# westlake-repl/PixelRec

Measured on AMD Instinct MI355X. Metric: user-sequences/sec at emb=512 seq_len=50 (SASRec IDNet training step: fwd+bwd+AdamW), higher is better.
Workload: dtype f32; 1 GPU; BASELINE.json configs[1]: SASRec IDNet emb=512 seq_len=50, 400001 items, 4 heads, inner 2x, 2 layers, BPR loss vs 1 sampled negative, dropout 0.1, AdamW lr 1e-4 wd 0.1; batch_per_gpu=64, global_batch=64, seq_len=50, n_items=400001, embedding_size=512, parallelism=dp1, hip_graph=True

## Files before the change

### pixelrec_amd/csrc/gemm_p3.hip

```cpp
#include "gemm_p4.cuh"

#include <cstdlib>

namespace pxr {

template <int EPI>
__device__ __forceinline__ float p3_epi_elem(float v, float bv, float av, float& aux_out, int act) {
  if constexpr (EPI == EPI_BIAS) {
    v += bv;
  } else if constexpr (EPI == EPI_BIAS_GELU) {
    v += bv;
    aux_out = v;
    v = gelu_erf(v);
  } else if constexpr (EPI == EPI_BIAS_GELU_GRAD) {
    v += bv;
    aux_out = dgelu_erf(v);
    v = gelu_erf(v);
  } else if constexpr (EPI == EPI_MUL) {
    v *= av;
  } else if constexpr (EPI == EPI_MUL_DGELU) {
    v *= dgelu_erf(av);
  } else if constexpr (EPI == EPI_ADD) {
    v += av;
  } else if constexpr (EPI == EPI_BIAS_ADD) {
// ... 105 lines not shown
        apre[it][4] = a1.x; apre[it][5] = a1.y; apre[it][6] = a1.z; apre[it][7] = a1.w;
      }
    }
  }
  float c_scale = 1.0f;
  if constexpr (Cfg::HALF) {
    const int ea = g.a_exp_dev ? *g.a_exp_dev : g.a_exp, eb = g.b_exp_dev ? *g.b_exp_dev : g.b_exp;
    const float sc = ldexpf(1.0f, -(ea + eb));
    if (g.c_exp_dev) c_scale = ldexpf(1.0f, *g.c_exp_dev);
#pragma unroll
    for (int i = 0; i < Cfg::TM; ++i)
#pragma unroll
      for (int j = 0; j < Cfg::TN; ++j)
#pragma unroll
        for (int e = 0; e < 16; ++e) accs.v[i][j][e] *= sc;
  }
  auto chunk = [&](int it, int row, int col, int nv, float (&v)[8]) __attribute__((always_inline)) {
    float bv[8], av[8], ao[8];
    const bool vec = vec_ok && nv == 8;
    if constexpr (EpiTraits<EPI>::HAS_BIAS) {
      if (vec) {
#pragma unroll
        for (int e = 0; e < 8; ++e) bv[e] = bpre[e];
      } else {
#pragma unroll
        for (int e = 0; e < 8; ++e) bv[e] = e < nv ? g.bias[col + e] : 0.f;
      }
    }
    if constexpr (EpiTraits<EPI>::READS_AUX) {
      const float* ap = g.aux + (int64_t)row * g.ldaux + col;
      if (vec) {
        if constexpr (PRE_AUX) {
#pragma unroll
          for (int e = 0; e < 8; ++e) av[e] = apre[it][e];
        } else {
          const float4 a0 = *reinterpret_cast<const float4*>(ap), a1 = *reinterpret_cast<const float4*>(ap + 4);
          av[0] = a0.x; av[1] = a0.y; av[2] = a0.z; av[3] = a0.w; av[4] = a1.x; av[5] = a1.y; av[6] = a1.z; av[7] = a1.w;
        }
      } else {
#pragma unroll
        for (int e = 0; e < 8; ++e) av[e] = e < nv ? ap[e] : 0.f;
      }
    }
#pragma unroll
    for (int e = 0; e < 8; ++e)
      v[e] = p3_epi_elem<EPI>(v[e], EpiTraits<EPI>::HAS_BIAS ? bv[e] : 0.f, EpiTraits<EPI>::READS_AUX ? av[e] : 0.f, ao[e], g.act);
    if (g.dbg & 16) return;
    if constexpr (P3EpiTraits<EPI>::WRITES_AUX) {
      float* ap = g.aux + (int64_t)row * g.ldaux + col;
      if (vec) {
        *reinterpret_cast<float4*>(ap) = make_float4(ao[0], ao[1], ao[2], ao[3]);
        *reinterpret_cast<float4*>(ap + 4) = make_float4(ao[4], ao[5], ao[6], ao[7]);
      } else {
#pragma unroll
        for (int e = 0; e < 8; ++e)
          if (e < nv) ap[e] = ao[e];
      }
    }
    if (g.C != nullptr) {
      float* cp = g.C + (int64_t)row * g.ldc + col;
      if (vec) {
        *reinterpret_cast<float4*>(cp) = make_float4(v[0], v[1], v[2], v[3]);
        *reinterpret_cast<float4*>(cp + 4) = make_float4(v[4], v[5], v[6], v[7]);
      } else {
#pragma unroll
        for (int e = 0; e < 8; ++e)
          if (e < nv) cp[e] = v[e];
      }
    }
    if (g.Cp.p != nullptr) {
      if constexpr (Cfg::HALF) {
#pragma unroll
        for (int e = 0; e < 8; ++e) v[e] *= c_scale;
      }
      px_store8(g.Cp, g.cp_fmt, g.status, row, col, v);
    }
  };
  if constexpr (PP) {
    p4_row_epilogue<Cfg>(accs, smem, g.M, g.N, m0, n0,
                         [&](int it, int row, int col, int nv) {
                           if (!(vec_ok && nv == 8)) return;
                           if constexpr (EpiTraits<EPI>::HAS_BIAS) {
                             if (it == 0) {
                               const float4 b0 = *reinterpret_cast<const float4*>(g.bias + col), b1 = *reinterpret_cast<const float4*>(g.bias + col + 4);
                               bpre[0] = b0.x; bpre[1] = b0.y; bpre[2] = b0.z; bpre[3] = b0.w; bpre[4] = b1.x; bpre[5] = b1.y; bpre[6] = b1.z; bpre[7] = b1.w;
                             }
                           }
                           if constexpr (PRE_AUX) {
                             const float* ap = g.aux + (int64_t)row * g.ldaux + col;
                             const float4 a0 = *reinterpret_cast<const float4*>(ap), a1 = *reinterpret_cast<const float4*>(ap + 4);
                             apre[it][0] = a0.x; apre[it][1] = a0.y; apre[it][2] = a0.z; apre[it][3] = a0.w;
                             apre[it][4] = a1.x; apre[it][5] = a1.y; apre[it][6] = a1.z; apre[it][7] = a1.w;
                           }
                         },
                         chunk);
  } else {
    p3_row_epilogue<Cfg>(accs, smem, g.M, g.N, m0, n0, chunk);
  }
}

__global__ void __launch_bounds__(256) split_planes_kernel(const float* __restrict__ x, int64_t ldx, int64_t rows, int cols8, P3Mat out,
                                                           int xcd) {
  const int64_t i = (int64_t)(xcd ? xcd_remap(blockIdx.x, gridDim.x) : blockIdx.x) * 256 + threadIdx.x;
  if (i >= rows * cols8) return;
  const int64_t row = i / cols8;
  const int c = (int)(i % cols8) * 8;
  const float4 a = *reinterpret_cast<const float4*>(x + row * ldx + c);
  const float4 b = *reinterpret_cast<const float4*>(x + row * ldx + c + 4);
  const float v[8] = {a.x, a.y, a.z, a.w, b.x, b.y, b.z, b.w};
  p3_store8(out, row, c, v);
}

struct P3DwProblem {
  P3Mat dy, x;
  float* dW;
  float* db;
  int T, N, K;
  int tile_begin, tiles_m;
  int dy_exp, x_exp;
  const int* dy_exp_dev;
  const int* x_exp_dev;
};
struct P3DwGroup {
  P3DwProblem p[DW_MAX];
  int n, total_tiles;
  unsigned* flags;
  unsigned* status;
};
int pxr_stream_flags(hipStream_t st, unsigned** flags, int* n_flags);
template <class Cfg, bool EARLY, int KS = 1>
__global__ void __launch_bounds__(Cfg::NT) grouped_dw_p3_kernel(const P3DwGroup g) {
  extern __shared__ __attribute__((aligned(16))) char smem[];
  static_assert(KS == 1 || (KS == 2 && Cfg::PINGPONG), "split-K: the ping-pong tiles");
  const int tl = xcd_remap(blockIdx.x, KS * g.total_tiles);
  const int t = tl / KS, half = tl % KS;
  int pi = 0;
#pragma unroll 1
  for (int i = 1; i < g.n; ++i)
    if (t >= g.p[i].tile_begin) pi = i;
  const P3DwProblem& P = g.p[pi];
  const int local = t - P.tile_begin;
  const int tm = local % P.tiles_m, tn = local / P.tiles_m;
  const int m0 = tm * Cfg::BM, n0 = tn * Cfg::BN;
  const int kpad = (P.T + 31) & ~31;
  typename Cfg::Acc accs;
  f32x16 ones_acc[Cfg::TM];
  const bool do_bias = (P.db != nullptr) && (tn == 0);
  if constexpr (KS == 2) {
    const int k0 = (kpad / 64) * 32;
    const int kb = half ? k0 : 0, kl = half ? kpad - k0 : k0;
    const P3Mat dyh{P.dy.p + (int64_t)kb * 32, P.dy.ps, P.dy.pr}, xh{P.x.p + (int64_t)kb * 32, P.x.ps, P.x.pr};
    if (do_bias) gemm_p4_mainloop<Cfg, false, false, true>(accs, dyh, xh, kl, m0, n0, smem, ones_acc);
    else gemm_p4_mainloop<Cfg, false, false, false>(accs, dyh, xh, kl, m0, n0, smem);
    if (half) {
      if (threadIdx.x == 0) {
        unsigned spins = 0;
        while (__hip_atomic_load(&g.flags[t], __ATOMIC_RELAXED, __HIP_MEMORY_SCOPE_AGENT) == 0u) {
          __builtin_amdgcn_s_sleep(4);
          if (++spins > (1u << 22)) {
            if (g.status) atomicOr(g.status, (unsigned)PXR_STATUS_GEMM_TIMEOUT);
            break;
          }
        }
      }
      __syncthreads();
    }
  } else if constexpr (Cfg::PINGPONG) {
    if (do_bias) gemm_p4_mainloop<Cfg, false, false, true>(accs, P.dy, P.x, kpad, m0, n0, smem, ones_acc);
    else gemm_p4_mainloop<Cfg, false, false, false>(accs, P.dy, P.x, kpad, m0, n0, smem);
  } else {
    if (do_bias) gemm_p3_mainloop<Cfg, false, false, EARLY, true>(accs, P.dy, P.x, kpad, m0, n0, smem, ones_acc);
    else gemm_p3_mainloop<Cfg, false, false, EARLY, false>(accs, P.dy, P.x, kpad, m0, n0, smem);
  }
  if constexpr (Cfg::HALF) {
    const int ey = P.dy_exp_dev ? *P.dy_exp_dev : P.dy_exp, ex = P.x_exp_dev ? *P.x_exp_dev : P.x_exp;
    const float sc = ldexpf(1.0f, -(ey + ex)), sb = ldexpf(1.0f, -ey);
#pragma unroll
    for (int i = 0; i < Cfg::TM; ++i) {
#pragma unroll
      for (int j = 0; j < Cfg::TN; ++j)
#pragma unroll
        for (int e = 0; e < 16; ++e) accs.v[i][j][e] *= sc;
      if (do_bias) {
#pragma unroll
        for (int e = 0; e < 16; ++e) ones_acc[i][e] *= sb;
      }
    }
  }
  float* dW = P.dW;
  const int64_t ldw = P.K;
  const bool vec_ok = (P.K % 8 == 0);
  constexpr int COH = (1 << 4) | 1;
  const bool add = (KS == 2) && half;
  const bool publish = (KS == 2) && !half;
  const bufrsrc rsw = make_rsrc(dW, (int64_t)P.N * P.K * 4);
  auto store = [&](int, int row, int col, int nv, float (&v)[8]) {
    float* cp = dW + (int64_t)row * ldw + col;
    const unsigned off = (unsigned)(((int64_t)row * ldw + col) * 4);
    if (vec_ok && nv == 8) {
      if (add) {
        const auto a = __builtin_amdgcn_raw_buffer_load_b128(rsw, off, 0, COH), b = __builtin_amdgcn_raw_buffer_load_b128(rsw, off + 16, 0, COH);
#pragma unroll
        for (int e = 0; e < 4; ++e) { v[e] += __uint_as_float(a[e]); v[4 + e] += __uint_as_float(b[e]); }
      }
      if (publish) {
        p3_u32x4 a, b;
#pragma unroll
        for (int e = 0; e < 4; ++e) { a[e] = __float_as_uint(v[e]); b[e] = __float_as_uint(v[4 + e]); }
        __builtin_amdgcn_raw_buffer_store_b128(a, rsw, off, 0, COH);
        __builtin_amdgcn_raw_buffer_store_b128(b, rsw, off + 16, 0, COH);
      } else {
        *reinterpret_cast<float4*>(cp) = make_float4(v[0], v[1], v[2], v[3]);
        *reinterpret_cast<float4*>(cp + 4) = make_float4(v[4], v[5], v[6], v[7]);
      }
    } else {
#pragma unroll
      for (int e = 0; e < 8; ++e)
        if (e < nv) {
          float o = v[e];
          if (add) o += __uint_as_float(__builtin_amdgcn_raw_buffer_load_b32(rsw, off + 4 * e, 0, COH));
          if (publish) __builtin_amdgcn_raw_buffer_store_b32(__float_as_uint(o), rsw, off + 4 * e, 0, COH);
          else cp[e] = o;
        }
    }
  };
  if constexpr (Cfg::PINGPONG) p4_row_epilogue<Cfg>(accs, smem, P.N, P.K, m0, n0, [](int, int, int, int) {}, store);
  else p3_row_epilogue<Cfg>(accs, smem, P.N, P.K, m0, n0, store);
  if (do_bias) {
    const int lane = threadIdx.x & 63, wave = threadIdx.x >> 6;
    const int wm = wave / Cfg::WGN, wn = wave % Cfg::WGN, h = lane >> 5, r = lane & 31;
    if (wn == 0 && r == 0) {
#pragma unroll
      for (int i = 0; i < Cfg::TM; ++i)
#pragma unroll
        for (int e = 0; e < 16; ++e) {
          const int row = m0 + wm * Cfg::WM + i * 32 + (e & 3) + 8 * (e >> 2) + 4 * h;
          if (row < P.N) {
            float o = ones_acc[i][e];
            if constexpr (KS == 2) {
              const bufrsrc rsb = make_rsrc(P.db, (int64_t)P.N * 4);
              if (add) o += __uint_as_float(__builtin_amdgcn_raw_buffer_load_b32(rsb, (unsigned)row * 4u, 0, COH));
              if (publish) __builtin_amdgcn_raw_buffer_store_b32(__float_as_uint(o), rsb, (unsigned)row * 4u, 0, COH);
              else P.db[row] = o;
            } else {
              P.db[row] = o;
            }
          }
        }
    }
  }
  if constexpr (KS == 2) {
    __builtin_amdgcn_s_waitcnt(0);
    __syncthreads();
    if (threadIdx.x == 0) __hip_atomic_store(&g.flags[t], half ? 0u : 1u, __ATOMIC_RELAXED, __HIP_MEMORY_SCOPE_AGENT);
  }
}

template <class Cfg, bool EARLY, int KS = 1>
static int launch_dw_p3(P3DwGroup& g, hipStream_t st) {
  int tiles = 0;
  for (int i = 0; i < g.n; ++i) {
    g.p[i].tile_begin = tiles;
    g.p[i].tiles_m = (g.p[i].N + Cfg::BM - 1) / Cfg::BM;
    tiles += g.p[i].tiles_m * ((g.p[i].K + Cfg::BN - 1) / Cfg::BN);
  }
  g.total_tiles = tiles;
  if constexpr (KS == 2) {
    if (2 * tiles > pxr_cu_count()) {
      pxr_set_error("pxr_grouped_dw_planes_f32: split-K needs both halves of its %d tiles resident at once, the device has %d CUs",
                    tiles, pxr_cu_count());
      return PXR_ERR_BAD_ARG;
    }
    int n_flags = 0;
    const int rc = pxr_stream_flags(st, &g.flags, &n_flags);
    if (rc != PXR_OK) return rc;
    if (tiles > n_flags) {
      pxr_set_error("pxr_grouped_dw_planes_f32: split-K launch with %d tiles (max %d)", tiles, n_flags);
      return PXR_ERR_BAD_ARG;
    }
    g.status = (unsigned*)pxr_status_word();
  }
  auto kern = grouped_dw_p3_kernel<Cfg, EARLY, KS>;
  static bool attr_set = false;
  if (!attr_set) {
    if (hipFuncSetAttribute(reinterpret_cast<const void*>(kern), hipFuncAttributeMaxDynamicSharedMemorySize, Cfg::LDS_BYTES) != hipSuccess) {
      (void)hipGetLastError();
      pxr_set_error("pxr_grouped_dw_planes_f32: cannot reserve %d bytes of LDS", Cfg::LDS_BYTES);
      return PXR_ERR_LAUNCH;
    }
    attr_set = true;
  }
  hipLaunchKernelGGL(kern, dim3((unsigned)(KS * tiles)), dim3(Cfg::NT), Cfg::LDS_BYTES, st, g);
  return pxr_check_launch("pxr_grouped_dw_planes_f32");
}

struct SplitMulti {
  const float* x[16]; int64_t ldx[16]; int rows[16], cols8[16]; P3Mat out[16];
  int64_t begin[17];
  int n;
  int fmt;
  float scale[16];
  int32_t* status;
};
__global__ void __launch_bounds__(256) split_planes_multi_kernel(const SplitMulti m) {
  const int64_t i = (int64_t)blockIdx.x * 256 + threadIdx.x;
  if (i >= m.begin[m.n]) return;
  int pi = 0;
#pragma unroll 1
  for (int k = 1; k < m.n; ++k)
    if (i >= m.begin[k]) pi = k;
  const int64_t li = i - m.begin[pi];
  const int64_t row = li / m.cols8[pi];
  const int c = (int)(li % m.cols8[pi]) * 8;
  const float* src = m.x[pi] + row * m.ldx[pi] + c;
  const float4 a = *reinterpret_cast<const float4*>(src);
  const float4 b = *reinterpret_cast<const float4*>(src + 4);
  float v[8] = {a.x, a.y, a.z, a.w, b.x, b.y, b.z, b.w};
  if (m.fmt == PXR_PLANES_H2) {
    const float sc = m.scale[pi];
#pragma unroll
    for (int e = 0; e < 8; ++e) v[e] *= sc;
  }
  px_store8(m.out[pi], m.fmt, m.status, row, c, v);
}

template <class Cfg, bool B_KC, int EPI, bool EARLY>
static int launch_p3(P3Args& g, hipStream_t st) {
  g.tiles_m = (g.M + Cfg::BM - 1) / Cfg::BM;
  g.tiles_n = (g.N + Cfg::BN - 1) / Cfg::BN;
  static const int xcd_env = getenv("PXR_GEMM_XCD") ? atoi(getenv("PXR_GEMM_XCD")) : -1;
  g.n_fastest = xcd_env >= 0 ? xcd_env : (g.M > g.N ? 1 : 0);
  static const int group_env = getenv("PXR_P3_GROUP_M") ? atoi(getenv("PXR_P3_GROUP_M")) : 0;
  g.group_m = (g.n_fastest && group_env > 1 && g.tiles_m >= 8 * group_env && g.tiles_n >= 4) ? group_env : 1;
  g.dbg = getenv("PXR_P3_DBG") ? atoi(getenv("PXR_P3_DBG")) : 0;
  auto kern = gemm_p3_kernel<Cfg, B_KC, EPI, EARLY>;
  static bool attr_set = false;
  if (!attr_set) {
    if (hipFuncSetAttribute(reinterpret_cast<const void*>(kern), hipFuncAttributeMaxDynamicSharedMemorySize, Cfg::LDS_BYTES) != hipSuccess) {
      (void)hipGetLastError();
      pxr_set_error("pxr_gemm_planes_f32: cannot reserve %d bytes of LDS", Cfg::LDS_BYTES);
      return PXR_ERR_LAUNCH;
    }
    attr_set = true;
  }
  hipLaunchKernelGGL(kern, dim3((unsigned)(g.tiles_m * g.tiles_n)), dim3(Cfg::NT), Cfg::LDS_BYTES, st, g);
  return pxr_check_launch("pxr_gemm_planes_f32");
}

template <class Cfg, bool EARLY>
static int epi_p3(int b_kc, int epilogue, P3Args& g, hipStream_t st) {
#define PXR_P3(BK_, E) \
  case E: return launch_p3<Cfg, BK_, E, EARLY>(g, st)
  if (b_kc) {
    switch (epilogue) {
      PXR_P3(true, EPI_NONE); PXR_P3(true, EPI_BIAS); PXR_P3(true, EPI_BIAS_GELU); PXR_P3(true, EPI_BIAS_GELU_GRAD);
      PXR_P3(true, EPI_BIAS_ACT_GRAD); PXR_P3(true, EPI_BIAS_ADD); PXR_P3(true, EPI_BIAS_QGELU); PXR_P3(true, EPI_BIAS_QGELU_GRAD);
      PXR_P3(true, EPI_BIAS_RELU);
    }
  } else {
    switch (epilogue) {
      PXR_P3(false, EPI_NONE); PXR_P3(false, EPI_ADD); PXR_P3(false, EPI_MUL);
    }
  }
#undef PXR_P3
  pxr_set_error("pxr_gemm_planes_f32: flavour b_kc=%d / epilogue %d is not instantiated", b_kc, epilogue);
  return PXR_ERR_BAD_ARG;
}

template <class Cfg>
static int epi_h2(int b_kc, int epilogue, P3Args& g, hipStream_t st) {
  if (b_kc) {
    switch (epilogue) {
      case EPI_NONE: return launch_p3<Cfg, true, EPI_NONE, false>(g, st);
      case EPI_BIAS: return launch_p3<Cfg, true, EPI_BIAS, false>(g, st);
      case EPI_BIAS_GELU: return launch_p3<Cfg, true, EPI_BIAS_GELU, false>(g, st);
      case EPI_BIAS_GELU_GRAD: return launch_p3<Cfg, true, EPI_BIAS_GELU_GRAD, false>(g, st);
      case EPI_BIAS_ACT_GRAD: return launch_p3<Cfg, true, EPI_BIAS_ACT_GRAD, false>(g, st);
      case EPI_BIAS_ADD: return launch_p3<Cfg, true, EPI_BIAS_ADD, false>(g, st);
      case EPI_BIAS_QGELU: return launch_p3<Cfg, true, EPI_BIAS_QGELU, false>(g, st);
      case EPI_BIAS_QGELU_GRAD: return launch_p3<Cfg, true, EPI_BIAS_QGELU_GRAD, false>(g, st);
      case EPI_BIAS_RELU: return launch_p3<Cfg, true, EPI_BIAS_RELU, false>(g, st);
    }
  } else {
    switch (epilogue) {
      case EPI_NONE: return launch_p3<Cfg, false, EPI_NONE, false>(g, st);
      case EPI_ADD: return launch_p3<Cfg, false, EPI_ADD, false>(g, st);
      case EPI_MUL: return launch_p3<Cfg, false, EPI_MUL, false>(g, st);
    }
  }
  pxr_set_error("pxr_gemm_h2_f32: flavour b_kc=%d / epilogue %d is not instantiated", b_kc, epilogue);
  return PXR_ERR_BAD_ARG;
}

}

using namespace pxr;

extern "C" int pxr_split_planes_f32(const float* x, int64_t rows, int64_t cols, int64_t ldx, void* planes, int64_t plane_stride,
                                    int64_t panel_rows, void* stream) {
  PXR_REQUIRE(x && planes, "pxr_split_planes_f32: null operand");
  PXR_REQUIRE(rows >= 0 && cols >= 0 && cols % 32 == 0 && ldx % 4 == 0, "pxr_split_planes_f32: cols must be a multiple of 32, ldx of 4");
  PXR_REQUIRE(panel_rows >= rows && panel_rows % 16 == 0 && plane_stride >= panel_rows * cols && plane_stride % 8 == 0,
              "pxr_split_planes_f32: panel_rows must be a multiple of 16 >= rows, plane_stride >= panel_rows * cols");
  PXR_REQUIRE((((uintptr_t)x | (uintptr_t)planes) & 15) == 0, "pxr_split_planes_f32: operands must be 16-byte aligned");
  const int64_t n = rows * (cols / 8);
  if (n == 0) return PXR_OK;
  PXR_REQUIRE((n + 255) / 256 < (1ll << 31), "pxr_split_planes_f32: too large");
  const P3Mat out{reinterpret_cast<__bf16*>(planes), plane_stride, panel_rows};
  const int xcd = getenv("PXR_SPLIT_XCD") ? atoi(getenv("PXR_SPLIT_XCD")) : 1;
  hipLaunchKernelGGL(split_planes_kernel, dim3((unsigned)((n + 255) / 256)), dim3(256), 0, (hipStream_t)stream, x, ldx, rows,
                     (int)(cols / 8), out, xcd);
  return pxr_check_launch("pxr_split_planes_f32");
}

extern "C" int pxr_split_planes_multi_f32(int n, const float* const* x, const int64_t* rows, const int64_t* cols, const int64_t* ldx,
                                          void* const* planes, const int64_t* plane_stride, const int64_t* panel_rows,
                                          void* stream) {
  PXR_REQUIRE(n >= 1 && n <= 16 && x && rows && cols && ldx && planes && plane_stride && panel_rows, "pxr_split_planes_multi_f32: bad args");
  SplitMulti m{};
  m.n = n;
  int64_t total = 0;
  for (int i = 0; i < n; ++i) {
    PXR_REQUIRE(x[i] && planes[i] && rows[i] > 0 && rows[i] < (1ll << 31) && cols[i] > 0 && cols[i] % 32 == 0 && ldx[i] % 4 == 0 &&
                    (((uintptr_t)x[i]) & 15) == 0 && p3_mat_ok(planes[i], plane_stride[i], panel_rows[i], rows[i], cols[i]),
                "pxr_split_planes_multi_f32: matrix %d is bad", i);
    m.x[i] = x[i]; m.ldx[i] = ldx[i]; m.rows[i] = (int)rows[i]; m.cols8[i] = (int)(cols[i] / 8);
    m.out[i] = P3Mat{reinterpret_cast<__bf16*>(planes[i]), plane_stride[i], panel_rows[i]};
    m.begin[i] = total;
    total += rows[i] * (cols[i] / 8);
  }
// ... 222 lines not shown
```

### pixelrec_amd/csrc/gemm_p4.cuh

```cuda
#pragma once
#include "gemm_p3.cuh"

namespace pxr {

template <int BM_, int BN_, int WGM_, int WGN_, int NS_, int NACC_, int DMA_ = 0, int NPL_ = 3, bool HALF_ = false>
struct P4Cfg {
  static constexpr int BM = BM_, BN = BN_, WGM = WGM_, WGN = WGN_, NS = NS_, NACC = NACC_, DMA = DMA_, NPL = NPL_;
  static constexpr bool HALF = HALF_;
  static_assert(NPL == 3 || NACC == 1 || (HALF && NACC == 2), "the reduced-product passes use one accumulator set");
  static_assert(!HALF || NPL == 2, "the fp16 format has two planes");
  static constexpr int G = WGM * WGN, NT = 64 * G, BK = 16;
  static constexpr int WM = BM / WGM, WN = BN / WGN, TM = WM / 32, TN = WN / 32;
  static constexpr int A_FR = BM / 32, B_FR = BN / 32;
  static constexpr int A_PIECES = NPL * A_FR, B_PIECES = NPL * B_FR;
  static constexpr int SLOT = (A_PIECES + B_PIECES) * 1024;
  static constexpr int RING_BYTES = NS * SLOT;
  static constexpr int EPI_COLS = BN > 128 ? 128 : BN, EPI_LD = EPI_COLS + 4, EPI_BYTES = BM * EPI_LD * 4;
  static constexpr int LDS_BYTES = RING_BYTES > EPI_BYTES ? RING_BYTES : EPI_BYTES;
  static constexpr bool PINGPONG = true;
  static_assert(G == 8, "two groups of four waves");
  static_assert(A_PIECES % 2 == 0 && B_PIECES % 2 == 0, "each group issues half of an operand's pieces");
  static_assert(WM % 32 == 0 && WN % 32 == 0 && TM >= 1 && TN >= 1, "wave tile = 32x32 blocks");
  static_assert(NS >= 3 && NS <= 8, "ring slots");
  static_assert(NACC == 1 || NACC == 2 || NACC == 3, "accumulator sets");
// ... 327 lines not shown
        for (int e = 0; e < 16; ++e) {
          if constexpr (NACC == 3) accs[i][j][e] += (accm[i][j][e] + accl[i][j][e]);
          else accs[i][j][e] += accm[i][j][e];
        }
  }
}

template <class Cfg, class TileFn>
__device__ __forceinline__ void gemm_p4_stream(const P3Mat& A, const P3Mat& B, int K, int m_first, int n0, int n_tiles, char* smem,
                                               TileFn&& done) {
  constexpr int TM = Cfg::TM, TN = Cfg::TN, NS = Cfg::NS, PF = NS - 1, NACC = Cfg::NACC;
  static_assert(Cfg::DMA == 0, "the stream issues its pieces in the L segments");
  using Loop = P4Loop<Cfg, true, true>;
  const int nkb = K / 16;
  const int total = n_tiles * nkb;
  if (total <= 0) return;
  typename Cfg::Acc acc;
  auto& accs = acc.v;
  f32x16 accm[NACC >= 2 ? TM : 1][TN], accl[NACC >= 3 ? TM : 1][TN];
  auto zero = [&]() {
#pragma unroll
    for (int i = 0; i < TM; ++i)
#pragma unroll
      for (int j = 0; j < TN; ++j)
#pragma unroll
        for (int e = 0; e < 16; ++e) {
          accs[i][j][e] = 0.f;
          if constexpr (NACC >= 2) accm[i][j][e] = 0.f;
          if constexpr (NACC >= 3) accl[i][j][e] = 0.f;
        }
  };
  zero();
  Loop L;
  L.init(A, B, m_first, n0, smem);
  int i_j = 0;
  unsigned i_tile_off = 0;
  auto issue_next = [&](int slot) {
    const unsigned sb = L.slot_addr(slot);
    L.opA.issue_at(i_j, sb, i_tile_off);
    L.opB.issue(i_j, sb);
    if (++i_j == nkb) { i_j = 0; i_tile_off += (unsigned)(Cfg::BM * 64); }
  };
#pragma unroll
  for (int s = 0; s < PF; ++s)
    if (s < total) issue_next(s);
  p4_wait_pieces(min(PF - 1, total - 1) * (L.opA.n + L.opB.n));
  __builtin_amdgcn_s_barrier();
  if (L.grp == 1) __builtin_amdgcn_s_barrier();
  typename Loop::Frag f;
  int slot = 0, islot = PF % NS, j = 0, tile = 0;
  bool pending = false;
  for (int it = 0; it < total; ++it) {
    if (pending) {
      if constexpr (NACC >= 2) {
#pragma unroll
        for (int i = 0; i < TM; ++i)
#pragma unroll
          for (int jj = 0; jj < TN; ++jj)
#pragma unroll
            for (int e = 0; e < 16; ++e) {
              if constexpr (NACC == 3) accs[i][jj][e] += (accm[i][jj][e] + accl[i][jj][e]);
              else accs[i][jj][e] += accm[i][jj][e];
            }
      }
      done(tile - 1, acc);
      zero();
      pending = false;
    }
    L.read_frag(f, slot);
    const bool more = it + PF < total;
    if (more) {
      issue_next(islot);
      L.wait_steady();
    } else {
      p3_wait_vm<0>();
    }
    asm volatile("s_waitcnt lgkmcnt(0)" ::: "memory");
    __builtin_amdgcn_sched_barrier(0);
    __builtin_amdgcn_s_barrier();
    __builtin_amdgcn_sched_barrier(0);
    __builtin_amdgcn_s_setprio(1);
    p4_mfma<Cfg, false>(f, accs, accm, accl, P4NoHook());
    __builtin_amdgcn_s_setprio(0);
    __builtin_amdgcn_sched_barrier(0);
    __builtin_amdgcn_s_barrier();
    __builtin_amdgcn_sched_barrier(0);
    slot = (slot + 1 == NS) ? 0 : slot + 1;
    if (more) islot = (islot + 1 == NS) ? 0 : islot + 1;
    if (++j == nkb) { j = 0; ++tile; pending = true; }
  }
  if (L.grp == 0) __builtin_amdgcn_s_barrier();
  if constexpr (NACC >= 2) {
#pragma unroll
    for (int i = 0; i < TM; ++i)
#pragma unroll
      for (int jj = 0; jj < TN; ++jj)
#pragma unroll
        for (int e = 0; e < 16; ++e) {
          if constexpr (NACC == 3) accs[i][jj][e] += (accm[i][jj][e] + accl[i][jj][e]);
          else accs[i][jj][e] += accm[i][jj][e];
        }
  }
  done(tile - 1, acc);
}

template <class Cfg>
struct P4ChunkMap {
  static constexpr int EC = Cfg::EPI_COLS, NP = Cfg::BN / EC, CPR = EC / 8, RPI = Cfg::NT / CPR, CPT = Cfg::BM / RPI;
};
template <class Cfg, class Pre, class Fn>
__device__ __forceinline__ void p4_row_epilogue(const typename Cfg::Acc& accs, char* smem, int M, int N, int m0, int n0, Pre&& pre, Fn&& fn) {
  static_assert(Cfg::EPI_OK, "epilogue chunk map");
  float* t = reinterpret_cast<float*>(smem);
  const int lane = threadIdx.x & 63, wave = __builtin_amdgcn_readfirstlane(threadIdx.x >> 6);
  const int wm = wave / Cfg::WGN, wn = wave % Cfg::WGN, h = lane >> 5, r = lane & 31;
  using Map = P4ChunkMap<Cfg>;
  constexpr int EC = Map::EC, NP = Map::NP, CPR = Map::CPR, RPI = Map::RPI, CPT = Map::CPT;
  const int c8 = (threadIdx.x % CPR) * 8;
#pragma unroll
  for (int pass = 0; pass < NP; ++pass) {
    const int col = n0 + pass * EC + c8;
#pragma unroll
    for (int it = 0; it < CPT; ++it) {
      const int row = it * RPI + threadIdx.x / CPR;
      if (m0 + row < M && col < N) pre(it, m0 + row, col, min(8, N - col));
    }
    if (pass) __syncthreads();
#pragma unroll
    for (int j = 0; j < Cfg::TN; ++j) {
      const int col0 = wn * Cfg::WN + j * 32 - pass * EC;
      if (col0 >= 0 && col0 < EC) {
#pragma unroll
        for (int i = 0; i < Cfg::TM; ++i)
#pragma unroll
          for (int e = 0; e < 16; ++e) {
            const int row = wm * Cfg::WM + i * 32 + (e & 3) + 8 * (e >> 2) + 4 * h;
            t[row * Cfg::EPI_LD + col0 + r] = accs.v[i][j][e];
          }
      }
    }
    __syncthreads();
#pragma unroll
    for (int it = 0; it < CPT; ++it) {
      const int row = it * RPI + threadIdx.x / CPR;
      if (m0 + row >= M || col >= N) continue;
      const float4 a = *reinterpret_cast<const float4*>(t + row * Cfg::EPI_LD + c8);
      const float4 b = *reinterpret_cast<const float4*>(t + row * Cfg::EPI_LD + c8 + 4);
      float v[8] = {a.x, a.y, a.z, a.w, b.x, b.y, b.z, b.w};
      fn(it, m0 + row, col, min(8, N - col), v);
    }
  }
}

}
```

Baseline: 84290 sequences/s.

## Symmetrize split-K dW reduction so both halves publish then add disjoint row blocks

Split-K weight-gradient tiles previously had one half publish the whole tile while the other half spun waiting and then added it. Now each half stages its accumulators in LDS, publishes one half of the rows, signals its own flag, waits for its partner's flag, and adds the partner's published rows into the other half. This balances the epilogue work across both workgroups and shortens the serialized wait. The cost is twice as many flags and a more intricate handshake in which both workgroups must be resident together.

```diff
diff --git a/pixelrec_amd/csrc/gemm_p3.hip b/pixelrec_amd/csrc/gemm_p3.hip
--- a/pixelrec_amd/csrc/gemm_p3.hip
+++ b/pixelrec_amd/csrc/gemm_p3.hip
@@ -281,19 +281,6 @@
     const P3Mat dyh{P.dy.p + (int64_t)kb * 32, P.dy.ps, P.dy.pr}, xh{P.x.p + (int64_t)kb * 32, P.x.ps, P.x.pr};
     if (do_bias) gemm_p4_mainloop<Cfg, false, false, true>(accs, dyh, xh, kl, m0, n0, smem, ones_acc);
     else gemm_p4_mainloop<Cfg, false, false, false>(accs, dyh, xh, kl, m0, n0, smem);
-    if (half) {
-      if (threadIdx.x == 0) {
-        unsigned spins = 0;
-        while (__hip_atomic_load(&g.flags[t], __ATOMIC_RELAXED, __HIP_MEMORY_SCOPE_AGENT) == 0u) {
-          __builtin_amdgcn_s_sleep(4);
-          if (++spins > (1u << 22)) {
-            if (g.status) atomicOr(g.status, (unsigned)PXR_STATUS_GEMM_TIMEOUT);
-            break;
-          }
-        }
-      }
-      __syncthreads();
-    }
   } else if constexpr (Cfg::PINGPONG) {
     if (do_bias) gemm_p4_mainloop<Cfg, false, false, true>(accs, P.dy, P.x, kpad, m0, n0, smem, ones_acc);
     else gemm_p4_mainloop<Cfg, false, false, false>(accs, P.dy, P.x, kpad, m0, n0, smem);
@@ -320,19 +307,19 @@
   const int64_t ldw = P.K;
   const bool vec_ok = (P.K % 8 == 0);
   constexpr int COH = (1 << 4) | 1;
-  const bool add = (KS == 2) && half;
-  const bool publish = (KS == 2) && !half;
+  constexpr int PLAIN = 0, PUBLISH = 1, ADD = 2;
   const bufrsrc rsw = make_rsrc(dW, (int64_t)P.N * P.K * 4);
-  auto store = [&](int, int row, int col, int nv, float (&v)[8]) {
+  auto store = [&](auto mode, int row, int col, int nv, float (&v)[8]) {
+    constexpr int MODE = decltype(mode)::value;
     float* cp = dW + (int64_t)row * ldw + col;
     const unsigned off = (unsigned)(((int64_t)row * ldw + col) * 4);
     if (vec_ok && nv == 8) {
-      if (add) {
+      if constexpr (MODE == ADD) {
         const auto a = __builtin_amdgcn_raw_buffer_load_b128(rsw, off, 0, COH), b = __builtin_amdgcn_raw_buffer_load_b128(rsw, off + 16, 0, COH);
 #pragma unroll
         for (int e = 0; e < 4; ++e) { v[e] += __uint_as_float(a[e]); v[4 + e] += __uint_as_float(b[e]); }
       }
-      if (publish) {
+      if constexpr (MODE == PUBLISH) {
         p3_u32x4 a, b;
 #pragma unroll
         for (int e = 0; e < 4; ++e) { a[e] = __float_as_uint(v[e]); b[e] = __float_as_uint(v[4 + e]); }
@@ -347,41 +334,66 @@
       for (int e = 0; e < 8; ++e)
         if (e < nv) {
           float o = v[e];
-          if (add) o += __uint_as_float(__builtin_amdgcn_raw_buffer_load_b32(rsw, off + 4 * e, 0, COH));
-          if (publish) __builtin_amdgcn_raw_buffer_store_b32(__float_as_uint(o), rsw, off + 4 * e, 0, COH);
+          if constexpr (MODE == ADD) o += __uint_as_float(__builtin_amdgcn_raw_buffer_load_b32(rsw, off + 4 * e, 0, COH));
+          if constexpr (MODE == PUBLISH) __builtin_amdgcn_raw_buffer_store_b32(__float_as_uint(o), rsw, off + 4 * e, 0, COH);
           else cp[e] = o;
         }
     }
   };
-  if constexpr (Cfg::PINGPONG) p4_row_epilogue<Cfg>(accs, smem, P.N, P.K, m0, n0, [](int, int, int, int) {}, store);
-  else p3_row_epilogue<Cfg>(accs, smem, P.N, P.K, m0, n0, store);
-  if (do_bias) {
+  auto bias = [&](auto mode) {
+    constexpr int MODE = decltype(mode)::value;
     const int lane = threadIdx.x & 63, wave = threadIdx.x >> 6;
     const int wm = wave / Cfg::WGN, wn = wave % Cfg::WGN, h = lane >> 5, r = lane & 31;
-    if (wn == 0 && r == 0) {
-#pragma unroll
-      for (int i = 0; i < Cfg::TM; ++i)
-#pragma unroll
-        for (int e = 0; e < 16; ++e) {
-          const int row = m0 + wm * Cfg::WM + i * 32 + (e & 3) + 8 * (e >> 2) + 4 * h;
-          if (row < P.N) {
-            float o = ones_acc[i][e];
-            if constexpr (KS == 2) {
-              const bufrsrc rsb = make_rsrc(P.db, (int64_t)P.N * 4);
-              if (add) o += __uint_as_float(__builtin_amdgcn_raw_buffer_load_b32(rsb, (unsigned)row * 4u, 0, COH));
-              if (publish) __builtin_amdgcn_raw_buffer_store_b32(__float_as_uint(o), rsb, (unsigned)row * 4u, 0, COH);
-              else P.db[row] = o;
-            } else {
-              P.db[row] = o;
-            }
-          }
+    if (wn != 0 || r != 0) return;
+    const bufrsrc rsb = make_rsrc(P.db, (int64_t)P.N * 4);
+#pragma unroll
+    for (int i = 0; i < Cfg::TM; ++i)
+#pragma unroll
+      for (int e = 0; e < 16; ++e) {
+        const int row = m0 + wm * Cfg::WM + i * 32 + (e & 3) + 8 * (e >> 2) + 4 * h;
+        if (row < P.N) {
+          float o = ones_acc[i][e];
+          if constexpr (MODE == ADD) o += __uint_as_float(__builtin_amdgcn_raw_buffer_load_b32(rsb, (unsigned)row * 4u, 0, COH));
+          if constexpr (MODE == PUBLISH) __builtin_amdgcn_raw_buffer_store_b32(__float_as_uint(o), rsb, (unsigned)row * 4u, 0, COH);
+          else P.db[row] = o;
         }
-    }
-  }
+      }
+  };
+  using Plain = std::integral_constant<int, PLAIN>;
+  using Publish = std::integral_constant<int, PUBLISH>;
+  using Add = std::integral_constant<int, ADD>;
   if constexpr (KS == 2) {
+    constexpr int HIT = P4ChunkMap<Cfg>::CPT / 2;
+    static_assert(P4ChunkMap<Cfg>::CPT % 2 == 0 && HIT * P4ChunkMap<Cfg>::RPI * 2 == Cfg::BM, "two row blocks of BM / 2 rows");
+    p4_stage_tile<Cfg>(accs, smem);
+    p4_walk_rows<Cfg, HIT>(smem, P.N, P.K, m0, n0, (1 - half) * HIT,
+                           [&](int row, int col, int nv, float (&v)[8]) { store(Publish{}, row, col, nv, v); });
+    if (do_bias && !half) bias(Publish{});
     __builtin_amdgcn_s_waitcnt(0);
     __syncthreads();
-    if (threadIdx.x == 0) __hip_atomic_store(&g.flags[t], half ? 0u : 1u, __ATOMIC_RELAXED, __HIP_MEMORY_SCOPE_AGENT);
+    if (threadIdx.x == 0) {
+      __hip_atomic_store(&g.flags[2 * t + half], 1u, __ATOMIC_RELAXED, __HIP_MEMORY_SCOPE_AGENT);
+      unsigned spins = 0;
+      while (__hip_atomic_load(&g.flags[2 * t + 1 - half], __ATOMIC_RELAXED, __HIP_MEMORY_SCOPE_AGENT) == 0u) {
+        __builtin_amdgcn_s_sleep(4);
+        if (++spins > (1u << 22)) {
+          if (g.status) atomicOr(g.status, (unsigned)PXR_STATUS_GEMM_TIMEOUT);
+          break;
+        }
+      }
+    }
+    __syncthreads();
+    p4_walk_rows<Cfg, HIT>(smem, P.N, P.K, m0, n0, half * HIT,
+                           [&](int row, int col, int nv, float (&v)[8]) { store(Add{}, row, col, nv, v); });
+    if (do_bias && half) bias(Add{});
+    __builtin_amdgcn_s_waitcnt(0);
+    __syncthreads();
+    if (threadIdx.x == 0) __hip_atomic_store(&g.flags[2 * t + 1 - half], 0u, __ATOMIC_RELAXED, __HIP_MEMORY_SCOPE_AGENT);
+  } else {
+    auto plain = [&](int, int row, int col, int nv, float (&v)[8]) { store(Plain{}, row, col, nv, v); };
+    if constexpr (Cfg::PINGPONG) p4_row_epilogue<Cfg>(accs, smem, P.N, P.K, m0, n0, [](int, int, int, int) {}, plain);
+    else p3_row_epilogue<Cfg>(accs, smem, P.N, P.K, m0, n0, plain);
+    if (do_bias) bias(Plain{});
   }
 }
 
@@ -403,8 +415,8 @@
     int n_flags = 0;
     const int rc = pxr_stream_flags(st, &g.flags, &n_flags);
     if (rc != PXR_OK) return rc;
-    if (tiles > n_flags) {
-      pxr_set_error("pxr_grouped_dw_planes_f32: split-K launch with %d tiles (max %d)", tiles, n_flags);
+    if (2 * tiles > n_flags) {
+      pxr_set_error("pxr_grouped_dw_planes_f32: split-K launch with %d tiles (max %d)", tiles, n_flags / 2);
       return PXR_ERR_BAD_ARG;
     }
     g.status = (unsigned*)pxr_status_word();
diff --git a/pixelrec_amd/csrc/gemm_p4.cuh b/pixelrec_amd/csrc/gemm_p4.cuh
--- a/pixelrec_amd/csrc/gemm_p4.cuh
+++ b/pixelrec_amd/csrc/gemm_p4.cuh
@@ -503,4 +503,38 @@
   }
 }
 
-}
+template <class Cfg>
+__device__ __forceinline__ void p4_stage_tile(const typename Cfg::Acc& accs, char* smem) {
+  static_assert(Cfg::EPI_OK && P4ChunkMap<Cfg>::NP == 1, "one epilogue pass");
+  float* t = reinterpret_cast<float*>(smem);
+  const int lane = threadIdx.x & 63, wave = __builtin_amdgcn_readfirstlane(threadIdx.x >> 6);
+  const int wm = wave / Cfg::WGN, wn = wave % Cfg::WGN, h = lane >> 5, r = lane & 31;
+#pragma unroll
+  for (int j = 0; j < Cfg::TN; ++j)
+#pragma unroll
+    for (int i = 0; i < Cfg::TM; ++i)
+#pragma unroll
+      for (int e = 0; e < 16; ++e) {
+        const int row = wm * Cfg::WM + i * 32 + (e & 3) + 8 * (e >> 2) + 4 * h;
+        t[row * Cfg::EPI_LD + wn * Cfg::WN + j * 32 + r] = accs.v[i][j][e];
+      }
+  __syncthreads();
+}
+template <class Cfg, int NIT, class Fn>
+__device__ __forceinline__ void p4_walk_rows(const char* smem, int M, int N, int m0, int n0, int it0, Fn&& fn) {
+  using Map = P4ChunkMap<Cfg>;
+  static_assert(Map::NP == 1 && NIT <= Map::CPT, "one epilogue pass");
+  const float* t = reinterpret_cast<const float*>(smem);
+  const int c8 = (threadIdx.x % Map::CPR) * 8, col = n0 + c8;
+#pragma unroll
+  for (int it = 0; it < NIT; ++it) {
+    const int row = (it0 + it) * Map::RPI + threadIdx.x / Map::CPR;
+    if (m0 + row >= M || col >= N) continue;
+    const float4 a = *reinterpret_cast<const float4*>(t + row * Cfg::EPI_LD + c8);
+    const float4 b = *reinterpret_cast<const float4*>(t + row * Cfg::EPI_LD + c8 + 4);
+    float v[8] = {a.x, a.y, a.z, a.w, b.x, b.y, b.z, b.w};
+    fn(m0 + row, col, min(8, N - col), v);
+  }
+}
+
+}
```

New measurement: 85280 sequences/s (median of 6 runs). +1.2%, better.
